# rballester/tntorch

Hardware: AMD Instinct MI355X
Metric: TT rounding 64^8 rank-64 -> rank-32 (round_tt rmax=32), cores/s, resident batch of 4096 trains per GPU (higher is better)
Workload: dtype f32

## Files before the change

include/ttround_hip.h:

```cpp
#ifndef TTROUND_HIP_H
#define TTROUND_HIP_H

#include <stdint.h>

#ifdef __cplusplus
extern "C" {
#endif

#define TTR_F32 0
#define TTR_F64 1

#define TTR_OK 0
#define TTR_E_INVALID (-1)
#define TTR_E_UNSUPPORTED (-2)
#define TTR_E_HIP (-3)
#define TTR_E_WORKSPACE (-4)

#define TTR_SCALE_NONE 0
#define TTR_SCALE_MUL 1
#define TTR_SCALE_DIV 2

#define TTR_EIG_RAW 0
#define TTR_EIG_REF 1
#define TTR_EIG_MATCH_DIAG 2
// ... 163 lines not shown
                   const void* sigma, int64_t stride_sigma, int left_ortho,
                   void* left, int64_t ldl, int64_t strideL,
                   void* right, int64_t ldr, int64_t strideR, void* stream);

int ttr_pow2_normalize(int dtype, int64_t count, int64_t batch, const void* x, int64_t stride_x,
                       void* out, int64_t stride_out, int32_t* e_out, int32_t* expo_acc, void* stream);

int ttr_scale_batch(int dtype, int64_t count, int64_t batch, const void* x, int64_t stride_x,
                    const void* scale, int64_t stride_scale, const int32_t* expo, int expo_sign,
                    void* out, int64_t stride_out, void* stream);

int64_t ttr_orth_fixup_workspace_bytes(int dtype, int64_t r, int64_t n, int64_t batch, int64_t elem_stride);
int ttr_orth_fixup(int dtype, int64_t r, int64_t n, int64_t batch, void* X, int64_t vec_stride, int64_t elem_stride,
                   int64_t strideX, const void* sigma, int64_t stride_sigma, double dead_rel, const int32_t* rank_dev,
                   void* workspace, int64_t workspace_bytes, void* stream);

#define TTR_ALG_SVD 0
#define TTR_ALG_EIG 1
int64_t ttr_round_tt_workspace_bytes(int dtype, int64_t N, const int64_t* shapes, const int64_t* rcap, int64_t batch,
                                     int eps_mode);
int ttr_round_tt(int dtype, int64_t N, const int64_t* shapes, int64_t batch, const void* const* cores_in, const int64_t* rcap,
                 int algorithm, int eps_mode, double eps, double flat_thr, int use_eigh_top, void* const* cores_out,
                 int32_t* ranks_dev, int32_t* zero_flag_dev, void* workspace, int64_t workspace_bytes, void* stream);

#define TTR_PROF_GEMM 0
#define TTR_PROF_QR_FACTOR 1
#define TTR_PROF_QR_APPLY 2
#define TTR_PROF_EIGH 3
#define TTR_PROF_MISC 4
#define TTR_PROF_ROTGRAM 5
#define TTR_PROF_PROJECT 6
#define TTR_PROF_ROWGRAM 7
#define TTR_PROF_NKINDS 8
int ttr_debug_set_qr_stamps(void* device_buffer);
#define TTR_KNOB_QR_PANEL 0
#define TTR_KNOB_BJ_INNER_SWEEPS 1
#define TTR_KNOB_GEMM_BIG 2
#define TTR_KNOB_QR_STAMP_BX 3
#define TTR_KNOB_QR_STAMP_BY 4
#define TTR_KNOB_QR_F64_NW4 5
#define TTR_KNOB_QR_RANK_SKIP 6
#define TTR_KNOB_QR_PACK 7
#define TTR_KNOB_RANK_NOISE_FLOOR 9
#define TTR_KNOB_ORTH_ROUNDS 10
#define TTR_KNOB_JACOBI_LIVE_WAVE 11
#define TTR_KNOB_ORTH_V2 12
#define TTR_KNOB_QR_INTERLEAVE 13
#define TTR_KNOB_SWEEP_STAGGER 14
#define TTR_KNOB_ORTH_SPLIT 15
#define TTR_KNOB_QR_STAGGER 16
#define TTR_KNOB_QR_PACK_PRE 17
#define TTR_KNOB_EIGH_BIG_OCC 18
#define TTR_KNOB_EIGH_SMALL 8
int ttr_debug_set_knob(int knob, int value);
int ttr_prof_enable(int on);
int ttr_prof_collect(double* ms, int64_t* launches);
int ttr_prof_collect_work(double* flops, double* bytes);


int64_t ttr_gather_chain_workspace_bytes(int dtype, int64_t nmodes, const int64_t* ranks, const int64_t* sizes, int64_t P,
                                         int64_t batch);
int ttr_gather_chain(int dtype, int64_t nmodes, int64_t batch, int64_t P, const int64_t* ranks, const int64_t* sizes,
                     const void* const* cores, const int64_t* core_strides, int idx_dtype, const void* const* idx,
                     const int64_t* idx_strides, void* out, int64_t stride_ob, int64_t stride_or, int64_t stride_op,
                     int64_t stride_oc, int64_t direct_max_points, void* oob_flag, void* workspace, int64_t workspace_bytes,
                     void* stream);

int ttr_gather_step(int dtype, int64_t P, int64_t rows_x, int64_t r, int64_t rn, int64_t I, const void* X, int64_t ldx,
                    const void* xrow, const void* G, int64_t gr, int64_t gi, int64_t gj, const void* idx, void* Y, int64_t ldy,
                    void* oob_flag, void* stream);

int64_t ttr_maxvol_workspace_bytes(int dtype, int64_t N, int64_t r, int64_t batch);
int ttr_maxvol(int dtype, int64_t batch, int64_t N, int64_t r, const void* A, int64_t stride_ab, double tol, int64_t max_iters,
               void* index, void* C, int64_t stride_cb, void* status, void* workspace, int64_t workspace_bytes, void* stream);

int64_t ttr_als_normal_groups(int64_t r0, int64_t r1);
int ttr_als_normal(int dtype, int64_t ntasks, int64_t r0, int64_t r1, const void* L, int64_t ldl, const void* R, int64_t ldr,
                   const void* w, const void* y, const void* perm, const void* task_begin, const void* task_end, void* Gp,
                   void* hp, void* stream);
int ttr_spd_solve(int dtype, int64_t n_items, int64_t K, const void* Gp, const void* hp, const void* part_off, int64_t part_base,
                  void* X, int64_t inner, int64_t s_item, int64_t s_a, int64_t s_b, void* Gsum, void* hsum, void* status,
                  const void* counts, void* stream);
int ttr_pinv_finish(int dtype, int64_t n_items, int64_t K, const void* V, const void* sigma, const void* t, const void* status,
                    void* X, int64_t inner, int64_t s_item, int64_t s_a, int64_t s_b, void* stream);

int64_t ttr_gather_grad_stage_rows(int dtype, int64_t r0, int64_t r1);
int64_t ttr_gather_grad_workspace_bytes(int dtype, int64_t ntasks, int64_t r0, int64_t r1);
int ttr_gather_grad(int dtype, int64_t I, int64_t ntasks, int64_t r0, int64_t r1, const void* L, int64_t ldl, const void* R,
                    int64_t ldr, const void* perm, const void* task_begin, const void* task_end, const void* task_off, void* dG,
                    void* workspace, int64_t workspace_bytes, void* stream);

int ttr_sparse_keys(int64_t P, int64_t N, const void* X, int64_t sx0, int64_t sx1, const void* shape, void* key, void* flag,
                    void* stream);
int ttr_sparse_levels(int64_t P, int64_t N, const void* X, int64_t sx0, int64_t sx1, const void* perm, void* lev, void* flag,
                      void* stream);
int64_t ttr_sparse_group_workspace_bytes(int64_t nb, int64_t I);
int ttr_sparse_group(int64_t nb, int64_t I, const void* blk_i, void* ilist, void* iptr, void* workspace, int64_t workspace_bytes,
                     void* stream);
int64_t ttr_sparse_gram_parts(int dtype, int64_t r, int64_t I, int64_t nb);
int64_t ttr_sparse_gram_workspace_bytes(int dtype, int64_t r, int64_t I, int64_t nb);
int ttr_sparse_gram(int dtype, int64_t r, int64_t I, int64_t nb, int64_t C, const void* colptr, const void* blk_i,
                    const void* blkcol, const void* ilist, const void* iptr, const void* V, int64_t ldv, void* G, int64_t ldg,
                    void* workspace, int64_t workspace_bytes, void* stream);
int ttr_sparse_project(int dtype, int64_t r, int64_t I, int64_t q, int64_t nb, int64_t C, const void* colptr, const void* blk_i,
                       const void* V, int64_t ldv, const void* U, int64_t su_row, int64_t su_col, void* W, int64_t ldw,
                       void* stream);
// ... 100 lines not shown
```

tntorch_amd/csrc/detail/ttr_internal.h:

```cpp
#pragma once
#include <type_traits>

#include "../ttr_common.h"

namespace ttr {

int gemm_dispatch(int dtype, int transA, int transB, int64_t M, int64_t N, int64_t K, const void* A, int64_t lda,
                  int64_t strideA, const void* B, int64_t ldb, int64_t strideB, void* C, int64_t ldc, int64_t strideC,
                  const void* rs, int64_t stride_rs, int rs_mode, const void* cs, int64_t stride_cs, int cs_mode,
                  int64_t batch, void* ws, int64_t ws_bytes, hipStream_t stream, int axpby = 0, double alpha = 1.0,
                  double beta = 0.0);
int64_t gemm_workspace_bytes(int dtype, int64_t M, int64_t N, int64_t K, int64_t batch);
int krp_contract_dispatch(int dtype, int64_t P, int64_t J, int64_t Q, int64_t R, const void* Tn, const void* B,
                          int64_t ldb, void* out, hipStream_t stream);
int hadamard_dispatch(int dtype, int64_t count, const void* a, const void* b, void* out, hipStream_t stream);
int core_kron_dispatch(int dtype, int64_t B, int64_t R1, int64_t S1, int64_t I, int64_t R2, int64_t S2, const void* a,
                       const void* c, void* out, hipStream_t stream);
int qr_factor_dispatch(int dtype, int64_t m, int64_t n, int64_t batch, const void* A, int64_t lda, int64_t strideA,
                       void* R, int64_t ldr, int64_t strideR, void* ws, int64_t ws_bytes, hipStream_t stream, int64_t a_cs = 1,
                       int32_t* expo_acc = nullptr);
int qr_apply_dispatch(int dtype, int64_t m, int64_t n, int64_t batch, void* ws, int64_t ws_bytes, const void* C,
                      int64_t ldc, int64_t strideC, int64_t kc, void* Out, int64_t ldo, int64_t strideO,
                      hipStream_t stream, int64_t o_cs = 1);
int64_t qr_workspace_bytes(int dtype, int64_t m, int64_t n, int64_t batch);
// ... 23 lines not shown
                        hipStream_t stream);
int bj_apply_dispatch(int dtype, int64_t b, int64_t npairs, int64_t items, void* G, int64_t ldg, int64_t strideG, void* V,
                      int64_t ldv, int64_t strideV, const int32_t* pair_tab, const void* W, const int32_t* ctrl, double* offsq,
                      hipStream_t stream);
int bj_control_dispatch(int dtype, int64_t items, int32_t* ctrl, double* state, const void* gnorm, int relative, double tol,
                        hipStream_t stream);
int64_t eigsel_scratch_bytes(int dtype, int64_t n, int64_t batch);
int eigsel_max_n();
int64_t tridiag_workspace_bytes(int dtype, int64_t n, int64_t batch);
int tridiag_dispatch(int dtype, int64_t n, int64_t batch, void* A, int64_t lda, int64_t strideA, void* d, void* e, void* tau,
                     void* ws, hipStream_t stream);
int eigsel_dispatch(int dtype, int64_t n, int64_t batch, int64_t k, const void* d, const void* e, void* lam, void* Z, void* scratch,
                    hipStream_t stream);
int tridiag_back_dispatch(int dtype, int64_t n, int64_t batch, int64_t k, const void* A, int64_t lda, int64_t strideA, const void* tau,
                          void* Z, hipStream_t stream);
int64_t eigh_workspace_bytes(int dtype, int64_t n, int64_t batch);
int eigh_max_n(int dtype);
int eigh_max_n_lds(int dtype);

int sweep_gram_parts(int64_t n, int64_t batch);
int sweep_gram_dispatch(int dtype, int64_t R, int64_t n, int64_t batch, const void* Mx, int64_t ldm, int64_t strideM,
                        const void* V1, int64_t ldv1, int64_t strideV1, void* G, int64_t nsplit, hipStream_t stream,
                        const int32_t* skip = nullptr, const int32_t* rows32 = nullptr);
int sweep_project_dispatch(int dtype, int64_t R, int64_t n, int64_t ro, int64_t batch, const void* Mx, int64_t ldm,
                           int64_t strideM, const void* V1, int64_t ldv1, int64_t strideV1, const void* V2, int64_t ldv2,
                           int64_t strideV2, const void* sigma, int64_t stride_sigma, int scale_right, void* right,
                           int64_t ldr, int64_t strideR, void* left, int64_t ldl, int64_t strideL, hipStream_t stream,
                           const int32_t* rows32 = nullptr);
int64_t qr_pushed_flag_offset(int dtype, int64_t I, int64_t n, int64_t batch);

int64_t colgram_workspace_bytes(int dtype, int64_t rows, int64_t n, int64_t batch);
int colgram_dispatch(int dtype, int64_t rows, int64_t n, int64_t batch, const void* Mx, int64_t ldm, int64_t strideM,
                     const void* V1, int64_t ldv1, int64_t strideV1, void* G, void* ws, int64_t ws_bytes, hipStream_t stream,
                     const int32_t* skip = nullptr);
int colproject_dispatch(int dtype, int64_t rows, int64_t n, int64_t ro, int64_t batch, const void* Mx, int64_t ldm,
                        int64_t strideM, const void* V1, int64_t ldv1, int64_t strideV1, const void* V2, int64_t ldv2,
                        int64_t strideV2, const void* sigma, int64_t stride_sigma, int left_ortho, void* left, int64_t ldl,
                        int64_t strideL, void* right, int64_t ldr, int64_t strideR, hipStream_t stream);

extern long long* g_qr_dbg;
extern int g_qr_variant;
extern int g_bj_inner_sweeps;
extern int g_gemm_big;
extern int g_qr_dbg_bx, g_qr_dbg_by;
extern int g_qr_f64_nw4;
extern int g_rank_skip_c;
extern int g_qr_pack;
extern int g_qr_interleave;
extern int g_qr_stagger;
extern int g_qr_pack_pre;
extern int g_qr_l1_idle;
extern int g_eigh_big_occ;
extern int g_sweep_stagger;
extern int g_rank_noise_c;
extern int g_jacobi_live_wave;
extern int g_eigh_small;
extern int g_orth_rounds, g_orth_v2, g_orth_split;

double* work_census_dev();

inline bool dtype_ok(int dtype) { return dtype == TTR_F32 || dtype == TTR_F64; }
inline int64_t elem_size(int dtype) { return dtype == TTR_F32 ? 4 : 8; }

template <typename F>
auto by_dtype(int dtype, F&& f) -> decltype(f(float{})) {
  if (dtype == TTR_F32) return f(float{});
  return f(double{});
}

inline bool contiguous(const int64_t* shape, const int64_t* strides, int nd) {
  int64_t want = 1;
  for (int d = nd - 1; d >= 0; --d) {
    if (shape[d] != 1 && strides[d] != want) return false;
    want *= shape[d];
  }
  return true;
}

inline bool aligned16(const void* p) { return ((uintptr_t)p & 15) == 0; }
inline int64_t align256(int64_t x) { return (x + 255) & ~int64_t(255); }

inline dim3 capped_grid(int64_t blocks) {
  const int64_t cap = 1 << 20;
  return dim3((unsigned)(blocks < cap ? blocks : cap));
}

template <typename T, typename F>
void by_pack_width(bool wide, F&& f) {
  if (wide) f(std::integral_constant<int, 16 / (int)sizeof(T)>{});
  else f(std::integral_constant<int, 1>{});
}

inline int core_check(const char* who, int dtype, int64_t R, int64_t I, int64_t C, const void* X, const int64_t* x_strides,
                      const void* out, const char* out_name, bool rest = true) {
  TTR_REQUIRE(dtype_ok(dtype), TTR_E_INVALID, "%s: bad dtype %d", who, dtype);
  TTR_REQUIRE(R >= 1 && I >= 1 && C >= 1, TTR_E_INVALID, "%s: bad sizes R = %lld, I = %lld, C = %lld", who, (long long)R, (long long)I,
              (long long)C);
  TTR_REQUIRE(X && x_strides && out && rest, TTR_E_INVALID, "%s: null pointer", who);
  TTR_REQUIRE(X != out, TTR_E_INVALID, "%s: X and %s must be different buffers", who, out_name);
  const int64_t xs[3] = {R, I, C};
  TTR_REQUIRE(contiguous(xs, x_strides, 3), TTR_E_UNSUPPORTED, "%s: X must be contiguous", who);
  TTR_REQUIRE((double)R * (double)I * (double)C < 9.0e18 / 64.0, TTR_E_UNSUPPORTED, "%s: core too large", who);
  return TTR_OK;
}

inline int strided_y_check(const char* who, int64_t R, int64_t I, int64_t C, const int64_t* y_strides, int64_t* sr, int64_t* si) {
// ... 10 lines not shown
```

tntorch_amd/csrc/ttr_api.hip:

```cpp
#include <stdarg.h>

#include <mutex>
#include <vector>

#include "detail/ttr_internal.h"

namespace ttr {

static thread_local std::string g_err;

void set_error(const char* fmt, ...) {
  char buf[512];
  va_list ap;
  va_start(ap, fmt);
  vsnprintf(buf, sizeof(buf), fmt, ap);
  va_end(ap);
  g_err = buf;
}

int hip_fail(hipError_t e, const char* what) {
  set_error("HIP error %d (%s) in %s", (int)e, hipGetErrorString(e), what);
  return TTR_E_HIP;
}

// ... 485 lines not shown
}

int ttr_krp_contract(int dtype, int64_t P, int64_t J, int64_t Q, int64_t R, const void* T, const void* B, int64_t ldb,
                     void* out, void* stream) {
  TTR_REQUIRE(dtype_ok(dtype), TTR_E_INVALID, "ttr_krp_contract: bad dtype %d", dtype);
  TTR_REQUIRE(P >= 0 && J >= 1 && Q >= 0 && R >= 1 && ldb >= R, TTR_E_INVALID, "ttr_krp_contract: bad sizes");
  if (P == 0 || Q == 0) return TTR_OK;
  TTR_REQUIRE(T && B && out, TTR_E_INVALID, "ttr_krp_contract: null pointer");
  return krp_contract_dispatch(dtype, P, J, Q, R, T, B, ldb, out, (hipStream_t)stream);
}

int ttr_hadamard(int dtype, int64_t count, const void* a, const void* b, void* out, void* stream) {
  TTR_REQUIRE(dtype_ok(dtype), TTR_E_INVALID, "ttr_hadamard: bad dtype %d", dtype);
  TTR_REQUIRE(count >= 0, TTR_E_INVALID, "ttr_hadamard: negative count");
  if (count == 0) return TTR_OK;
  TTR_REQUIRE(a && b && out, TTR_E_INVALID, "ttr_hadamard: null pointer");
  return hadamard_dispatch(dtype, count, a, b, out, (hipStream_t)stream);
}

int ttr_core_kron(int dtype, int64_t batch, int64_t R1, int64_t S1, int64_t I, int64_t R2, int64_t S2, const void* a,
                  const void* c, void* out, void* stream) {
  TTR_REQUIRE(dtype_ok(dtype), TTR_E_INVALID, "ttr_core_kron: bad dtype %d", dtype);
  TTR_REQUIRE(batch >= 0 && R1 >= 1 && S1 >= 1 && I >= 1 && R2 >= 1 && S2 >= 1, TTR_E_INVALID, "ttr_core_kron: bad sizes");
  if (batch == 0) return TTR_OK;
  TTR_REQUIRE(a && c && out, TTR_E_INVALID, "ttr_core_kron: null pointer");
  return core_kron_dispatch(dtype, batch, R1, S1, I, R2, S2, a, c, out, (hipStream_t)stream);
}

int ttr_debug_set_qr_stamps(void* device_buffer) {
  g_qr_dbg = (long long*)device_buffer;
  return TTR_OK;
}

int ttr_debug_set_knob(int knob, int value) {
  switch (knob) {
    case TTR_KNOB_QR_STAMP_BX:
      g_qr_dbg_bx = value;
      return TTR_OK;
    case TTR_KNOB_QR_STAMP_BY:
      g_qr_dbg_by = value;
      return TTR_OK;
    case TTR_KNOB_EIGH_SMALL:
      TTR_REQUIRE(value >= 0 && value <= 3, TTR_E_INVALID, "ttr_debug_set_knob: small-eigensolver switch %d outside [0, 3]", value);
      g_eigh_small = value;
      return TTR_OK;
    case TTR_KNOB_ORTH_SPLIT:
      TTR_REQUIRE(value >= 0 && value <= 65535, TTR_E_INVALID, "ttr_debug_set_knob: orth split threshold %d outside [0, 65535]", value);
      g_orth_split = value;
      return TTR_OK;
    case TTR_KNOB_SWEEP_STAGGER:
      TTR_REQUIRE(value >= 0 && value <= 2, TTR_E_INVALID, "ttr_debug_set_knob: stagger mode %d outside [0, 2]", value);
      g_sweep_stagger = value;
      return TTR_OK;
    case TTR_KNOB_EIGH_BIG_OCC:
      TTR_REQUIRE(value == 0 || value == 2 || value == 3, TTR_E_INVALID, "ttr_debug_set_knob: eigensolver occupancy %d not in {0, 2, 3}", value);
      g_eigh_big_occ = value;
      return TTR_OK;
    case TTR_KNOB_QR_PACK_PRE:
      TTR_REQUIRE(value >= 0 && value <= 3, TTR_E_INVALID, "ttr_debug_set_knob: pack-flag switch %d outside [0, 3]", value);
      g_qr_pack_pre = value & 1;
      g_qr_l1_idle = (value & 2) ? 0 : 1;
      return TTR_OK;
    case TTR_KNOB_QR_STAGGER:
      TTR_REQUIRE(value >= 0 && value <= 1024, TTR_E_INVALID, "ttr_debug_set_knob: stagger of %d kilo-cycles outside [0, 1024]", value);
      g_qr_stagger = value;
      return TTR_OK;
    case TTR_KNOB_QR_INTERLEAVE:
      TTR_REQUIRE(value >= 0 && value <= 1, TTR_E_INVALID, "ttr_debug_set_knob: interleave switch %d outside [0, 1]", value);
      g_qr_interleave = value;
      return TTR_OK;
    case TTR_KNOB_ORTH_V2:
      TTR_REQUIRE(value >= 0 && value <= 2, TTR_E_INVALID, "ttr_debug_set_knob: orth_fixup variant %d outside [0, 2]", value);
      g_orth_v2 = value;
      return TTR_OK;
    case TTR_KNOB_JACOBI_LIVE_WAVE:
      TTR_REQUIRE(value >= 0 && value <= 1, TTR_E_INVALID, "ttr_debug_set_knob: pass-2 Jacobi switch %d outside [0, 1]", value);
      g_jacobi_live_wave = value;
      return TTR_OK;
    case TTR_KNOB_ORTH_ROUNDS:
      TTR_REQUIRE(value >= 1 && value <= 4, TTR_E_INVALID, "ttr_debug_set_knob: %d rounds outside [1, 4]", value);
      g_orth_rounds = value;
      return TTR_OK;
    case TTR_KNOB_RANK_NOISE_FLOOR:
      TTR_REQUIRE(value >= 0 && value <= 1024, TTR_E_INVALID, "ttr_debug_set_knob: rank-rule noise floor %d outside [0, 1024]", value);
      g_rank_noise_c = value;
      return TTR_OK;
    case TTR_KNOB_QR_PACK:
      TTR_REQUIRE(value >= 0 && value <= 3, TTR_E_INVALID, "ttr_debug_set_knob: packing switch %d outside [0, 3]", value);
      g_qr_pack = value;
      return TTR_OK;
    case TTR_KNOB_QR_RANK_SKIP:
      TTR_REQUIRE(value >= 0 && value <= 4096, TTR_E_INVALID, "ttr_debug_set_knob: rank-skip factor %d outside [0, 4096]", value);
      g_rank_skip_c = value;
      return TTR_OK;
    case TTR_KNOB_QR_F64_NW4:
      TTR_REQUIRE(value >= 0 && value <= 7, TTR_E_INVALID, "ttr_debug_set_knob: 4-wave block switch %d outside [0, 7]", value);
      g_qr_f64_nw4 = value;
      return TTR_OK;
    case TTR_KNOB_GEMM_BIG:
      TTR_REQUIRE(value >= 0 && value <= 1, TTR_E_INVALID, "ttr_debug_set_knob: big-tile GEMM switch %d outside [0, 1]", value);
      g_gemm_big = value;
      return TTR_OK;
    case TTR_KNOB_BJ_INNER_SWEEPS:
      TTR_REQUIRE(value >= 0 && value <= 64, TTR_E_INVALID, "ttr_debug_set_knob: %d inner sweeps outside [0, 64]", value);
      g_bj_inner_sweeps = value;
      return TTR_OK;
// ... 57 lines not shown
```

tntorch_amd/csrc/ttr_sweep.hip:

```cpp
#include <type_traits>

#include "detail/ttr_internal.h"

namespace ttr {

constexpr int KLD = 80;

template <typename T>
struct SweepArgs {
  int R;
  int64_t n;
  const T* M;
  int64_t ldm, strideM;
  const T* V1;
  int64_t ldv1, strideV1;
  T* G;
  int nsplit;
  const int32_t* skip;
  const int32_t* rows32;
  const T* V2;
  int64_t ldv2, strideV2;
  const T* sigma;
  int64_t stride_sigma;
  int ro;
// ... 103 lines not shown
#pragma unroll
      for (int ks = 0; ks < 16; ++ks) {
        const int k = 4 * ks + g;
        a[ks] = (k < Rl && c0 + cl < p.n) ? Mp[(int64_t)k * p.ldm + c0 + cl] : T(0);
      }
    };
    const int64_t nsteps = ce > cb + wave ? (ce - cb - wave + 3) / 4 : 0;
    const int64_t rot = (p.stagger >= 2 && nsteps > 1) ? (int64_t)(b % nsteps) : 0;
    auto step_c = [&](int64_t sidx) { int64_t sq = sidx + rot; if (sq >= nsteps) sq -= nsteps; return cb + wave + 4 * sq; };
    T a[16], an[16];
    if (nsteps > 0) load_cols(step_c(0), a);
    for (int64_t sidx = 0; sidx < nsteps; ++sidx) {
      const bool more = sidx + 1 < nsteps;
      if (more) load_cols(step_c(sidx + 1), an);
      Acc mw[4];
#pragma unroll
      for (int t = 0; t < 4; ++t) {
        mw[t] = M::zero();
#pragma unroll
        for (int ks = 0; ks < 16; ++ks) mw[t] = M::mma(a[ks], Vl[(4 * ks + g) * KLD + 16 * t + cl], mw[t]);
      }
      gram_update(mw);
      if (more) {
#pragma unroll
        for (int ks = 0; ks < 16; ++ks) a[ks] = an[ks];
      }
    }
  }
  __syncthreads();
#pragma unroll
  for (int i = 0; i < 10; ++i)
#pragma unroll
    for (int r = 0; r < 4; ++r) smem[(wave * 10 + i) * 256 + lane * 4 + r] = G[i][r];
  __syncthreads();
  T* __restrict__ Gout = p.G + ((int64_t)b * p.nsplit + split) * R * R;
  for (int idx = tid; idx < 10 * 256; idx += kThreads) {
    const int tile = idx >> 8, e = idx & 255, ln = e >> 2, r = e & 3;
    const T v = (smem[idx] + smem[2560 + idx]) + (smem[5120 + idx] + smem[7680 + idx]);
    int ti = 0, rem = tile;
    while (rem >= 4 - ti) { rem -= 4 - ti; ++ti; }
    const int tj = ti + rem;
    const int row = 16 * ti + M::row(ln, r), col = 16 * tj + (ln & 15);
    if (row < R && col < R) {
      Gout[row * R + col] = v;
      if (ti != tj) Gout[col * R + row] = v;
    }
  }
}

constexpr int V1LD = 82;
constexpr int UBLK = 16 * V1LD;
__device__ __forceinline__ int urow(int k) { return (k >> 4) * UBLK + (k & 15) * KLD; }

template <typename T>
__global__ __launch_bounds__(kThreads, (sizeof(T) == 4 ? 4 : 1)) void project_kernel(SweepArgs<T> p) {
  using M = Mfma<T>;
  using Acc = typename M::Acc;
  constexpr int V2LD = 72;
  __shared__ __attribute__((aligned(16))) T V2l[64 * V2LD];
  __shared__ __attribute__((aligned(16))) T V1l[64 * V1LD];
  T* Ul = V1l;
  __shared__ T isg[64];
  const int tid = threadIdx.x, lane = tid & 63, wave = tid >> 6, cl = lane & 15, g = lane >> 4;
  const int64_t b = blockIdx.y;
  const int split = blockIdx.x;
  const T* __restrict__ Mp = p.M + b * p.strideM;
  const int R = p.R, ro = p.ro;
  const int nt = (ro + 15) / 16;
  const T* __restrict__ V2 = p.V2 + b * p.strideV2;
  const T* __restrict__ sg = p.sigma ? p.sigma + b * p.stride_sigma : nullptr;
  T* __restrict__ Lo = (p.left && split == 0) ? p.left + b * p.strideL : nullptr;
  for (int idx = tid; idx < 64 * 64; idx += kThreads) {
    const int m = idx >> 6, i = idx & 63;
    V2l[m * V2LD + i] = (m < R && i < ro) ? V2[(int64_t)m * p.ldv2 + i] : T(0);
  }
  if (tid < 64) {
    T sc = T(1);
    if (p.scale_right && sg && tid < ro) {
      const T x = sg[tid];
      sc = (fabs((double)x) < (double)Num<T>::tiny()) ? T(0) : T(1) / x;
    }
    isg[tid] = sc;
  }
  if (p.V1) {
    const T* __restrict__ V1 = p.V1 + b * p.strideV1;
    for (int idx = tid; idx < 64 * 64; idx += kThreads) {
      const int k = idx >> 6, m = idx & 63;
      V1l[k * V1LD + m] = (k < R && m < R) ? V1[(int64_t)k * p.ldv1 + m] : T(0);
    }
    __syncthreads();
    Acc u0 = M::zero(), u1 = M::zero(), u2 = M::zero(), u3 = M::zero();
#pragma unroll
    for (int ks = 0; ks < 16; ++ks) {
      const T a = V1l[(16 * wave + cl) * V1LD + 4 * ks + g];
      u0 = M::mma(a, V2l[(4 * ks + g) * V2LD + cl], u0);
      u1 = M::mma(a, V2l[(4 * ks + g) * V2LD + 16 + cl], u1);
      u2 = M::mma(a, V2l[(4 * ks + g) * V2LD + 32 + cl], u2);
      u3 = M::mma(a, V2l[(4 * ks + g) * V2LD + 48 + cl], u3);
    }
#pragma unroll
    for (int r = 0; r < 4; ++r) {
      T* dst = Ul + urow(16 * wave + M::row(lane, r)) + cl;
      dst[0] = u0[r];
      dst[16] = u1[r];
      dst[32] = u2[r];
      dst[48] = u3[r];
    }
  } else {
// ... 39 lines not shown
#pragma unroll
        for (int u = 0; u < SL; ++u) bm[u][ks] = x.v[u];
      }
#pragma unroll
      for (int t = 0; t < 4; ++t) {
        if (t < nt) {
          Acc acc[SL];
#pragma unroll
          for (int u = 0; u < SL; ++u) acc[u] = M::zero();
#pragma unroll
          for (int ks = 0; ks < NK; ++ks) {
            const T af = Ul[urow(4 * ks + g) + 16 * t + cl];
#pragma unroll
            for (int u = 0; u < SL; ++u) acc[u] = M::mma(af, bm[u][ks], acc[u]);
          }
#pragma unroll
          for (int r = 0; r < 4; ++r) {
            const int row = 16 * t + M::row(lane, r);
            if (row < ro && lim > 0) {
              const T sc = isg[row];
              T* dst = Ro + (int64_t)row * p.ldr + col;
              if (al && lim >= SL) {
                typedef T VT __attribute__((ext_vector_type(SL)));
                VT o;
#pragma unroll
                for (int u = 0; u < SL; ++u) o[u] = acc[u][r] * sc;
                *reinterpret_cast<VT*>(dst) = o;
              } else {
#pragma unroll
                for (int u = 0; u < SL; ++u)
                  if (u < lim) dst[u] = acc[u][r] * sc;
              }
            }
          }
        }
      }
    }
  };
  using I2 = std::integral_constant<int, 2>;
  using I4 = std::integral_constant<int, 4>;
  using I8 = std::integral_constant<int, 8>;
  using I16 = std::integral_constant<int, 16>;
  if (Rl <= 32) {
#ifdef TTR_PROJECT_WIDE
    if (al4) main_loop(I8{}, I4{});
    else
#endif
      main_loop(I8{}, I2{});
  } else {
    main_loop(I16{}, I2{});
  }
  (void)al4;
}

constexpr int CLD = 68;

template <typename T>
struct ColArgs {
  int64_t rows;
  int n;
  const T* M;
  int64_t ldm, strideM;
  const T* V1;
  int64_t ldv1, strideV1;
  T* G;
  int nsplit;
  const int32_t* skip;
  const T* V2;
  int64_t ldv2, strideV2;
  const T* sigma;
  int64_t stride_sigma;
  int ro;
  int left_ortho;
  T* left;
  int64_t ldl, strideL;
  T* right;
  int64_t ldr, strideR;
};

template <typename T, bool ROT>
__global__ __launch_bounds__(kThreads, (sizeof(T) == 4 ? (ROT ? 3 : 4) : 1)) void colgram_kernel(ColArgs<T> p) {
  using M = Mfma<T>;
  using Acc = typename M::Acc;
  constexpr int RED = 4 * 10 * 256;
  constexpr int VSZ = 64 * CLD;
  __shared__ __attribute__((aligned(16))) T smem[RED > VSZ ? RED : VSZ];
  T* Vl = smem;
  const int tid = threadIdx.x, lane = tid & 63, wave = tid >> 6, cl = lane & 15, g = lane >> 4;
  const int64_t b = blockIdx.y;
  if (p.skip && p.skip[b] != 0) return;
  const int split = blockIdx.x;
  const T* __restrict__ Mp = p.M + b * p.strideM;
  const int n = p.n;
  if constexpr (ROT) {
    const T* __restrict__ V1 = p.V1 + b * p.strideV1;
    for (int idx = tid; idx < 64 * 64; idx += kThreads) {
      const int k = idx >> 6, j = idx & 63;
      Vl[k * CLD + j] = (k < n && j < n) ? V1[(int64_t)k * p.ldv1 + j] : T(0);
    }
    __syncthreads();
  }
  Acc G[10];
#pragma unroll
  for (int i = 0; i < 10; ++i) G[i] = M::zero();
  int64_t cb, ce;
  split_range((p.rows + 15) / 16, p.nsplit, split, cb, ce);
// ... 253 lines not shown

int colgram_dispatch(int dtype, int64_t rows, int64_t n, int64_t batch, const void* Mx, int64_t ldm, int64_t strideM,
                     const void* V1, int64_t ldv1, int64_t strideV1, void* G, void* ws, int64_t ws_bytes, hipStream_t stream,
                     const int32_t* skip) {
  TTR_REQUIRE(n >= 1 && n <= 64, TTR_E_UNSUPPORTED, "ttr_colgram: %lld columns (the fused kernels hold <= 64)", (long long)n);
  if (dtype == TTR_F32) return colgram_typed<float>(rows, n, batch, Mx, ldm, strideM, V1, ldv1, strideV1, G, ws, ws_bytes, stream, skip);
  return colgram_typed<double>(rows, n, batch, Mx, ldm, strideM, V1, ldv1, strideV1, G, ws, ws_bytes, stream, skip);
}

template <typename T>
static int colproject_typed(int64_t rows, int64_t n, int64_t ro, int64_t batch, const void* Mx, int64_t ldm, int64_t strideM,
                            const void* V1, int64_t ldv1, int64_t strideV1, const void* V2, int64_t ldv2, int64_t strideV2,
                            const void* sigma, int64_t stride_sigma, int left_ortho, void* left, int64_t ldl,
                            int64_t strideL, void* right, int64_t ldr, int64_t strideR, hipStream_t stream) {
  ColArgs<T> p{};
  p.rows = rows; p.n = (int)n; p.M = (const T*)Mx; p.ldm = ldm; p.strideM = strideM;
  p.V1 = (const T*)V1; p.ldv1 = ldv1; p.strideV1 = strideV1;
  p.V2 = (const T*)V2; p.ldv2 = ldv2; p.strideV2 = strideV2;
  p.sigma = (const T*)sigma; p.stride_sigma = stride_sigma; p.ro = (int)ro; p.left_ortho = left_ortho;
  p.left = (T*)left; p.ldl = ldl; p.strideL = strideL;
  p.right = (T*)right; p.ldr = ldr; p.strideR = strideR;
  p.nsplit = col_split(rows, batch);
  ProfScope prof(TTR_PROF_PROJECT, stream);
  for (int64_t b0 = 0; b0 < batch; b0 += 65535) {
    const int64_t nb = batch - b0 < 65535 ? batch - b0 : 65535;
    ColArgs<T> q = p;
    q.M = p.M + b0 * strideM;
    if (V1) q.V1 = p.V1 + b0 * strideV1;
    q.V2 = p.V2 + b0 * strideV2;
    if (sigma) q.sigma = p.sigma + b0 * stride_sigma;
    q.left = p.left + b0 * strideL;
    if (right) q.right = p.right + b0 * strideR;
    if (q.V1) hipLaunchKernelGGL((colproject_kernel<T, true>), dim3((unsigned)p.nsplit, (unsigned)nb), dim3(kThreads), 0, stream, q);
    else hipLaunchKernelGGL((colproject_kernel<T, false>), dim3((unsigned)p.nsplit, (unsigned)nb), dim3(kThreads), 0, stream, q);
  }
  TTR_HIP_CHECK(hipGetLastError());
  return TTR_OK;
}

int colproject_dispatch(int dtype, int64_t rows, int64_t n, int64_t ro, int64_t batch, const void* Mx, int64_t ldm,
                        int64_t strideM, const void* V1, int64_t ldv1, int64_t strideV1, const void* V2, int64_t ldv2,
                        int64_t strideV2, const void* sigma, int64_t stride_sigma, int left_ortho, void* left, int64_t ldl,
                        int64_t strideL, void* right, int64_t ldr, int64_t strideR, hipStream_t stream) {
  TTR_REQUIRE(n >= 1 && n <= 64 && ro >= 1 && ro <= n, TTR_E_UNSUPPORTED,
              "ttr_colproject: %lld columns / %lld kept (the fused kernel holds <= 64 columns)", (long long)n, (long long)ro);
  if (dtype == TTR_F32)
    return colproject_typed<float>(rows, n, ro, batch, Mx, ldm, strideM, V1, ldv1, strideV1, V2, ldv2, strideV2, sigma,
                                   stride_sigma, left_ortho, left, ldl, strideL, right, ldr, strideR, stream);
  return colproject_typed<double>(rows, n, ro, batch, Mx, ldm, strideM, V1, ldv1, strideV1, V2, ldv2, strideV2, sigma,
                                  stride_sigma, left_ortho, left, ldl, strideL, right, ldr, strideR, stream);
}

int g_sweep_stagger = 1;

static int pick_split(int64_t n, int64_t batch) {
  const int64_t chunks = (n + 31) / 32;
  int64_t want = (2048 + batch - 1) / batch;
  int64_t maxs = chunks / 8;
  if (maxs < 1) maxs = 1;
  int64_t s = want < maxs ? want : maxs;
  if (s > 64) s = 64;
  return (int)(s < 1 ? 1 : s);
}

int sweep_gram_parts(int64_t n, int64_t batch) { return pick_split(n, batch); }

template <typename T>
static int gram_typed(int64_t R, int64_t n, int64_t batch, const void* Mx, int64_t ldm, int64_t strideM, const void* V1,
                      int64_t ldv1, int64_t strideV1, void* G, int64_t nsplit, hipStream_t stream, const int32_t* skip,
                      const int32_t* rows32) {
  SweepArgs<T> p{};
  p.skip = skip;
  p.rows32 = rows32;
  p.R = (int)R; p.n = n; p.M = (const T*)Mx; p.ldm = ldm; p.strideM = strideM;
  p.V1 = (const T*)V1; p.ldv1 = ldv1; p.strideV1 = strideV1;
  p.G = (T*)G; p.nsplit = (int)nsplit;
  p.stagger = g_sweep_stagger;
  if (work_census_on()) {
    const double s = (double)sizeof(T), sym = 10.0 / 16.0;
    auto gr = [&](double Re) { return 2.0 * Re * Re * (double)n * sym + (V1 ? 2.0 * (double)R * Re * (double)n : 0.0); };
    const double fl[4] = {gr((double)R), gr(R > 32 ? 32.0 : (double)R), 0.0, 0.0};
    const double by[4] = {s * R * (double)n, s * (R > 32 ? 32.0 : (double)R) * (double)n, 0.0, 0.0};
    work_items(V1 ? TTR_PROF_ROTGRAM : TTR_PROF_ROWGRAM, rows32, skip, batch, fl, by, stream);
  }
  ProfScope prof(V1 ? TTR_PROF_ROTGRAM : TTR_PROF_ROWGRAM, stream);
  for (int64_t b0 = 0; b0 < batch; b0 += 65535) {
    const int64_t nb = batch - b0 < 65535 ? batch - b0 : 65535;
    SweepArgs<T> q = p;
    q.M = p.M + b0 * strideM;
    if (V1) q.V1 = p.V1 + b0 * strideV1;
    q.G = p.G + b0 * nsplit * R * R;
    if (skip) q.skip = skip + b0;
    if (rows32) q.rows32 = rows32 + b0;
    const dim3 grid((unsigned)nsplit, (unsigned)nb);
    if (V1) hipLaunchKernelGGL((rotgram_kernel<T, false>), grid, dim3(kThreads), 0, stream, q);
    else hipLaunchKernelGGL((rotgram_kernel<T, true>), grid, dim3(kThreads), 0, stream, q);
  }
  TTR_HIP_CHECK(hipGetLastError());
  return TTR_OK;
}

int sweep_gram_dispatch(int dtype, int64_t R, int64_t n, int64_t batch, const void* Mx, int64_t ldm, int64_t strideM,
                        const void* V1, int64_t ldv1, int64_t strideV1, void* G, int64_t nsplit, hipStream_t stream,
                        const int32_t* skip, const int32_t* rows32) {
  TTR_REQUIRE(R >= 1 && R <= 64, TTR_E_UNSUPPORTED, "ttr_rowgram / ttr_rotgram: %lld rows (the fused kernels hold <= 64)",
              (long long)R);
  TTR_REQUIRE(nsplit >= 1 && nsplit <= 65535, TTR_E_INVALID, "ttr_rowgram / ttr_rotgram: bad split %lld", (long long)nsplit);
  if (dtype == TTR_F32) return gram_typed<float>(R, n, batch, Mx, ldm, strideM, V1, ldv1, strideV1, G, nsplit, stream, skip, rows32);
  return gram_typed<double>(R, n, batch, Mx, ldm, strideM, V1, ldv1, strideV1, G, nsplit, stream, skip, rows32);
}

template <typename T>
static int project_typed(int64_t R, int64_t n, int64_t ro, int64_t batch, const void* Mx, int64_t ldm, int64_t strideM,
                         const void* V1, int64_t ldv1, int64_t strideV1, const void* V2, int64_t ldv2, int64_t strideV2,
                         const void* sigma, int64_t stride_sigma, int scale_right, void* right, int64_t ldr,
                         int64_t strideR, void* left, int64_t ldl, int64_t strideL, hipStream_t stream, const int32_t* rows32) {
  SweepArgs<T> p{};
  p.rows32 = rows32;
  p.R = (int)R; p.n = n; p.M = (const T*)Mx; p.ldm = ldm; p.strideM = strideM;
  p.V1 = (const T*)V1; p.ldv1 = ldv1; p.strideV1 = strideV1;
  p.V2 = (const T*)V2; p.ldv2 = ldv2; p.strideV2 = strideV2;
  p.sigma = (const T*)sigma; p.stride_sigma = stride_sigma; p.ro = (int)ro; p.scale_right = scale_right;
  p.right = (T*)right; p.ldr = ldr; p.strideR = strideR;
  p.left = (T*)left; p.ldl = ldl; p.strideL = strideL;
  p.nsplit = pick_split(n, batch);
  p.stagger = g_sweep_stagger;
  if (work_census_on()) {
    const double s = (double)sizeof(T), Re = R > 32 ? 32.0 : (double)R;
    const double fl[4] = {2.0 * R * (double)ro * (double)n, 2.0 * Re * (double)ro * (double)n, 0.0, 0.0};
    const double by[4] = {s * (R + ro) * (double)n, s * (Re + ro) * (double)n, 0.0, 0.0};
    work_items(TTR_PROF_PROJECT, rows32, nullptr, batch, fl, by, stream);
  }
  ProfScope prof(TTR_PROF_PROJECT, stream);
  for (int64_t b0 = 0; b0 < batch; b0 += 65535) {
    const int64_t nb = batch - b0 < 65535 ? batch - b0 : 65535;
    SweepArgs<T> q = p;
    q.M = p.M + b0 * strideM;
    if (V1) q.V1 = p.V1 + b0 * strideV1;
    q.V2 = p.V2 + b0 * strideV2;
    if (sigma) q.sigma = p.sigma + b0 * stride_sigma;
    q.right = p.right + b0 * strideR;
    if (left) q.left = p.left + b0 * strideL;
    if (rows32) q.rows32 = rows32 + b0;
    hipLaunchKernelGGL(project_kernel<T>, dim3((unsigned)p.nsplit, (unsigned)nb), dim3(kThreads), 0, stream, q);
  }
  TTR_HIP_CHECK(hipGetLastError());
  return TTR_OK;
}

int sweep_project_dispatch(int dtype, int64_t R, int64_t n, int64_t ro, int64_t batch, const void* Mx, int64_t ldm,
                           int64_t strideM, const void* V1, int64_t ldv1, int64_t strideV1, const void* V2, int64_t ldv2,
                           int64_t strideV2, const void* sigma, int64_t stride_sigma, int scale_right, void* right,
                           int64_t ldr, int64_t strideR, void* left, int64_t ldl, int64_t strideL, hipStream_t stream,
                           const int32_t* rows32) {
  TTR_REQUIRE(R >= 1 && R <= 64 && ro >= 1 && ro <= R, TTR_E_UNSUPPORTED,
              "ttr_project: %lld rows / %lld kept (the fused kernel holds <= 64 rows)", (long long)R, (long long)ro);
  if (dtype == TTR_F32)
    return project_typed<float>(R, n, ro, batch, Mx, ldm, strideM, V1, ldv1, strideV1, V2, ldv2, strideV2, sigma,
                                stride_sigma, scale_right, right, ldr, strideR, left, ldl, strideL, stream, rows32);
  return project_typed<double>(R, n, ro, batch, Mx, ldm, strideM, V1, ldv1, strideV1, V2, ldv2, strideV2, sigma,
                               stride_sigma, scale_right, right, ldr, strideR, left, ldl, strideL, stream, rows32);
}

}
```

Before: 1.438 million.

## Add lean rows32-specialized gram and project kernels with higher occupancy

Adds specialized fp32 kernels for batch items flagged rows32 (effective rank at most 32): a gram kernel that accumulates only the 32x32 block with a register prefetch pipeline, and a projection kernel that keeps only 32 columns of the rotation. Both declare launch bounds of 8 blocks per unit. The existing general kernels are still launched afterwards but skip the items the lean kernels already handled. The aim is to cut wasted MFMA work and register pressure on reduced-rank items, at the cost of an extra launch per stage and more code paths.

```diff
diff --git a/include/ttround_hip.h b/include/ttround_hip.h
--- a/include/ttround_hip.h
+++ b/include/ttround_hip.h
@@ -239,6 +239,7 @@
 #define TTR_KNOB_QR_PACK_PRE 17
 #define TTR_KNOB_EIGH_BIG_OCC 18
 #define TTR_KNOB_EIGH_SMALL 8
+#define TTR_KNOB_SWEEP_LEAN 19
 int ttr_debug_set_knob(int knob, int value);
 int ttr_prof_enable(int on);
 int ttr_prof_collect(double* ms, int64_t* launches);
diff --git a/tntorch_amd/csrc/detail/ttr_internal.h b/tntorch_amd/csrc/detail/ttr_internal.h
--- a/tntorch_amd/csrc/detail/ttr_internal.h
+++ b/tntorch_amd/csrc/detail/ttr_internal.h
@@ -99,6 +99,7 @@
 extern int g_qr_l1_idle;
 extern int g_eigh_big_occ;
 extern int g_sweep_stagger;
+extern int g_sweep_lean;
 extern int g_rank_noise_c;
 extern int g_jacobi_live_wave;
 extern int g_eigh_small;
diff --git a/tntorch_amd/csrc/ttr_api.hip b/tntorch_amd/csrc/ttr_api.hip
--- a/tntorch_amd/csrc/ttr_api.hip
+++ b/tntorch_amd/csrc/ttr_api.hip
@@ -561,6 +561,10 @@
       TTR_REQUIRE(value >= 0 && value <= 2, TTR_E_INVALID, "ttr_debug_set_knob: stagger mode %d outside [0, 2]", value);
       g_sweep_stagger = value;
       return TTR_OK;
+    case TTR_KNOB_SWEEP_LEAN:
+      TTR_REQUIRE(value >= 0 && value <= 1, TTR_E_INVALID, "ttr_debug_set_knob: lean sweep switch %d outside [0, 1]", value);
+      g_sweep_lean = value;
+      return TTR_OK;
     case TTR_KNOB_EIGH_BIG_OCC:
       TTR_REQUIRE(value == 0 || value == 2 || value == 3, TTR_E_INVALID, "ttr_debug_set_knob: eigensolver occupancy %d not in {0, 2, 3}", value);
       g_eigh_big_occ = value;
diff --git a/tntorch_amd/csrc/ttr_sweep.hip b/tntorch_amd/csrc/ttr_sweep.hip
--- a/tntorch_amd/csrc/ttr_sweep.hip
+++ b/tntorch_amd/csrc/ttr_sweep.hip
@@ -179,8 +179,11 @@
 constexpr int UBLK = 16 * V1LD;
 __device__ __forceinline__ int urow(int k) { return (k >> 4) * UBLK + (k & 15) * KLD; }
 
-template <typename T>
+template <typename T, bool REST = false>
 __global__ __launch_bounds__(kThreads, (sizeof(T) == 4 ? 4 : 1)) void project_kernel(SweepArgs<T> p) {
+  if constexpr (REST) {
+    if (p.rows32[blockIdx.y] != 0) return;
+  }
   using M = Mfma<T>;
   using Acc = typename M::Acc;
   constexpr int V2LD = 72;
@@ -326,6 +329,243 @@
   }
   (void)al4;
 }
+
+constexpr int kLeanAhead = 3;
+
+template <typename T>
+__global__ __launch_bounds__(kThreads, 8) void rowgram_rows32_kernel(SweepArgs<T> p) {
+  using M = Mfma<T>;
+  using Acc = typename M::Acc;
+  __shared__ __attribute__((aligned(16))) T red[4 * 3 * 256];
+  static_assert(std::is_same<T, float>::value, "slab loads and the write-out below assume the fp32 accumulator layout");
+  const int tid = threadIdx.x, lane = tid & 63, cl = lane & 15, g = lane >> 4;
+  const int wave = __builtin_amdgcn_readfirstlane(tid >> 6);
+  const int64_t b = blockIdx.y;
+  if (p.rows32[b] == 0) return;
+  const int split = blockIdx.x;
+  const T* __restrict__ Mp = p.M + b * p.strideM;
+  Acc G[3];
+#pragma unroll
+  for (int i = 0; i < 3; ++i) G[i] = M::zero();
+  const bool al = ((p.ldm & 3) == 0) && ((reinterpret_cast<uintptr_t>(Mp) & (4 * sizeof(T) - 1)) == 0);
+  int64_t cb, ce;
+  split_range((p.n + 15) / 16, p.nsplit, split, cb, ce);
+  auto gram_update = [&](const Acc (&mw)[2]) {
+#pragma unroll
+    for (int r = 0; r < 4; ++r) G[0] = M::mma(mw[0][r], mw[0][r], G[0]);
+#pragma unroll
+    for (int r = 0; r < 4; ++r) G[1] = M::mma(mw[0][r], mw[1][r], G[1]);
+#pragma unroll
+    for (int r = 0; r < 4; ++r) G[2] = M::mma(mw[1][r], mw[1][r], G[2]);
+  };
+  const int64_t nsteps = ce > cb + wave ? (ce - cb - wave + 3) / 4 : 0;
+  const int64_t rot = (p.stagger >= 2 && nsteps > 1) ? (int64_t)(b % nsteps) : 0;
+  auto step_c = [&](int64_t sidx) { int64_t sq = sidx + rot; if (sq >= nsteps) sq -= nsteps; return cb + wave + 4 * sq; };
+  constexpr int NS = kLeanAhead + 1;
+  auto run = [&](auto WIDEC) {
+    constexpr bool WIDE = decltype(WIDEC)::value;
+    auto load_slab = [&](int64_t c, Acc (&mw)[2]) {
+      const int64_t col = c * 16 + 4 * g;
+#pragma unroll
+      for (int t = 0; t < 2; ++t) {
+        const T* src = Mp + (int64_t)(16 * t + cl) * p.ldm + col;
+        if constexpr (WIDE) {
+          mw[t] = *reinterpret_cast<const Acc*>(src);
+        } else {
+          const Pack<T, 4> x = load_pack<T, 4>(src, al, p.n - col);
+#pragma unroll
+          for (int r = 0; r < 4; ++r) mw[t][r] = x.v[r];
+        }
+      }
+    };
+    Acc slab[NS][2];
+    int64_t s0 = 0;
+    if (nsteps >= NS + kLeanAhead) {
+#pragma unroll
+      for (int d = 0; d < kLeanAhead; ++d) load_slab(step_c(d), slab[d]);
+      do {
+#pragma unroll
+        for (int u = 0; u < NS; ++u) {
+          load_slab(step_c(s0 + u + kLeanAhead), slab[(u + kLeanAhead) % NS]);
+          __builtin_amdgcn_sched_barrier(0);
+          gram_update(slab[u]);
+          __builtin_amdgcn_sched_barrier(0);
+        }
+        s0 += NS;
+      } while (s0 + NS + kLeanAhead <= nsteps);
+    } else {
+#pragma unroll
+      for (int d = 0; d < kLeanAhead; ++d)
+        if (d < nsteps) load_slab(step_c(d), slab[d]);
+    }
+    for (; s0 < nsteps; s0 += NS) {
+#pragma unroll
+      for (int u = 0; u < NS; ++u) {
+        const int64_t sidx = s0 + u;
+        if (sidx < nsteps) {
+          if (sidx + kLeanAhead < nsteps) load_slab(step_c(sidx + kLeanAhead), slab[(u + kLeanAhead) % NS]);
+          gram_update(slab[u]);
+        }
+      }
+    }
+  };
+  if (al && ce * 16 <= p.n) run(std::true_type{});
+  else run(std::false_type{});
+#pragma unroll
+  for (int i = 0; i < 3; ++i)
+#pragma unroll
+    for (int r = 0; r < 4; ++r) red[(wave * 3 + i) * 256 + lane * 4 + r] = G[i][r];
+  __syncthreads();
+  T* __restrict__ Gout = p.G + ((int64_t)b * p.nsplit + split) * 64 * 64;
+  for (int idx = tid; idx < 64 * 64; idx += kThreads) {
+    const int row = idx >> 6, col = idx & 63;
+    T v = T(0);
+    if (row < 32 && col < 32) {
+      const bool low = row >= 16 && col < 16;
+      const int i = (low ? col : row) & 15, j = (low ? row : col) & 15;
+      const int tile = (row >> 4) + (col >> 4);
+      const int e = tile * 256 + ((i >> 2) * 16 + j) * 4 + (i & 3);
+      v = (red[e] + red[768 + e]) + (red[1536 + e] + red[2304 + e]);
+    }
+    Gout[idx] = v;
+  }
+}
+
+constexpr int ULD = 48;
+
+template <typename T>
+__global__ __launch_bounds__(kThreads, 8) void project_rows32_kernel(SweepArgs<T> p) {
+  using M = Mfma<T>;
+  using Acc = typename M::Acc;
+  __shared__ __attribute__((aligned(16))) T Wl[64 * ULD];
+  __shared__ T isg[32];
+  static_assert(std::is_same<T, float>::value, "the store addresses below assume the fp32 accumulator layout");
+  const int tid = threadIdx.x, lane = tid & 63, cl = lane & 15, g = lane >> 4;
+  const int wave = __builtin_amdgcn_readfirstlane(tid >> 6);
+  const int64_t b = blockIdx.y;
+  if (p.rows32[b] == 0) return;
+  const int split = blockIdx.x;
+  const T* __restrict__ Mp = p.M + b * p.strideM;
+  const int ro = p.ro;
+  const int nt = (ro + 15) / 16;
+  const T* __restrict__ V2 = p.V2 + b * p.strideV2;
+  const T* __restrict__ sg = p.sigma ? p.sigma + b * p.stride_sigma : nullptr;
+  T* __restrict__ Lo = (p.left && split == 0) ? p.left + b * p.strideL : nullptr;
+  for (int idx = tid; idx < 64 * 32; idx += kThreads) {
+    const int m = idx >> 5, i = idx & 31;
+    Wl[m * ULD + i] = (i < ro) ? V2[(int64_t)m * p.ldv2 + i] : T(0);
+  }
+  if (tid < 32) {
+    T sc = T(1);
+    if (p.scale_right && sg && tid < ro) {
+      const T x = sg[tid];
+      sc = (fabs((double)x) < (double)Num<T>::tiny()) ? T(0) : T(1) / x;
+    }
+    isg[tid] = sc;
+  }
+  if (p.V1) {
+    const T* __restrict__ V1 = p.V1 + b * p.strideV1 + (int64_t)(16 * wave + cl) * p.ldv1 + g;
+    T a[16];
+#pragma unroll
+    for (int ks = 0; ks < 16; ++ks) a[ks] = V1[4 * ks];
+    __syncthreads();
+    Acc u0 = M::zero(), u1 = M::zero();
+#pragma unroll
+    for (int ks = 0; ks < 16; ++ks) {
+      u0 = M::mma(a[ks], Wl[(4 * ks + g) * ULD + cl], u0);
+      u1 = M::mma(a[ks], Wl[(4 * ks + g) * ULD + 16 + cl], u1);
+    }
+    __syncthreads();
+#pragma unroll
+    for (int r = 0; r < 4; ++r) {
+      T* dst = Wl + (16 * wave + M::row(lane, r)) * ULD + cl;
+      dst[0] = u0[r];
+      dst[16] = u1[r];
+    }
+  }
+  __syncthreads();
+  if (Lo) {
+    for (int idx = tid; idx < 64 * ro; idx += kThreads) {
+      const int k = idx / ro, i = idx - k * ro;
+      const T u = Wl[k * ULD + i];
+      Lo[(int64_t)k * p.ldl + i] = (p.scale_right && sg) ? u * sg[i] : u;
+    }
+  }
+  T af[2][8];
+#pragma unroll
+  for (int t = 0; t < 2; ++t)
+#pragma unroll
+    for (int ks = 0; ks < 8; ++ks) af[t][ks] = Wl[(4 * ks + g) * ULD + 16 * t + cl];
+  T* __restrict__ Ro = p.right + b * p.strideR;
+  const bool al = ((p.ldm & 1) == 0) && ((p.ldr & 1) == 0) && ((reinterpret_cast<uintptr_t>(Mp) & (2 * sizeof(T) - 1)) == 0) &&
+                  ((reinterpret_cast<uintptr_t>(Ro) & (2 * sizeof(T) - 1)) == 0);
+  int64_t cb, ce;
+  split_range((p.n + 31) / 32, p.nsplit, split, cb, ce);
+  const int64_t col_b = cb * 32, col_e = ce * 32 < p.n ? ce * 32 : p.n;
+  const int64_t nch = (col_e - col_b + 31) / 32;
+  const int64_t nsteps = nch > wave ? (nch - wave + 3) / 4 : 0;
+  const int64_t rot = (p.stagger && nsteps > 1) ? (int64_t)(b % nsteps) : 0;
+  const T* __restrict__ Mg = Mp + (int64_t)g * p.ldm;
+  T* __restrict__ Rg = Ro + (int64_t)M::row(lane, 0) * p.ldr;
+  typedef T VT __attribute__((ext_vector_type(2)));
+  auto step = [&](auto WHOLEC, const T* mk, T* rk, int64_t lim) {
+    constexpr bool WHOLE = decltype(WHOLEC)::value;
+    T bm[2][8];
+#pragma unroll
+    for (int ks = 0; ks < 8; ++ks) {
+      const T* src = mk + (int64_t)(4 * ks) * p.ldm;
+      if constexpr (WHOLE) {
+        const VT x = *reinterpret_cast<const VT*>(src);
+        bm[0][ks] = x[0];
+        bm[1][ks] = x[1];
+      } else {
+        const Pack<T, 2> x = load_pack<T, 2>(src, al, lim > 0 ? lim : 0);
+        bm[0][ks] = x.v[0];
+        bm[1][ks] = x.v[1];
+      }
+    }
+#pragma unroll
+    for (int t = 0; t < 2; ++t) {
+      if (t < nt) {
+        Acc acc[2] = {M::zero(), M::zero()};
+#pragma unroll
+        for (int ks = 0; ks < 8; ++ks) {
+#pragma unroll
+          for (int u = 0; u < 2; ++u) acc[u] = M::mma(af[t][ks], bm[u][ks], acc[u]);
+        }
+#pragma unroll
+        for (int r = 0; r < 4; ++r) {
+          const int row = 16 * t + M::row(lane, r);
+          if (row < ro && (WHOLE || lim > 0)) {
+            const T sc = isg[row];
+            T* dst = rk + (int64_t)(16 * t + r) * p.ldr;
+            if (WHOLE || (al && lim >= 2)) {
+              VT o;
+              o[0] = acc[0][r] * sc;
+              o[1] = acc[1][r] * sc;
+              *reinterpret_cast<VT*>(dst) = o;
+            } else {
+              dst[0] = acc[0][r] * sc;
+              if (lim > 1) dst[1] = acc[1][r] * sc;
+            }
+          }
+        }
+      }
+    }
+  };
+  for (int64_t sidx = 0; sidx < nsteps; ++sidx) {
+    int64_t sq = sidx + rot;
+    if (sq >= nsteps) sq -= nsteps;
+    const int64_t cw = col_b + (wave + 4 * sq) * 32;
+    int64_t col = cw + 2 * cl;
+    asm volatile("" : "+v"(col));
+    const T* mk = Mg + col;
+    T* rk = Rg + col;
+    if (al && cw + 32 <= col_e) step(std::true_type{}, mk, rk, 2);
+    else step(std::false_type{}, mk, rk, col_e - col);
+  }
+}
+
 
 constexpr int CLD = 68;
 
@@ -685,6 +925,8 @@
 }
 
 int g_sweep_stagger = 1;
+int g_sweep_lean = 1;
+constexpr int64_t kLeanMinItems = 256;
 
 static int pick_split(int64_t n, int64_t batch) {
   const int64_t chunks = (n + 31) / 32;
@@ -726,6 +968,12 @@
     if (skip) q.skip = skip + b0;
     if (rows32) q.rows32 = rows32 + b0;
     const dim3 grid((unsigned)nsplit, (unsigned)nb);
+    if constexpr (std::is_same<T, float>::value) {
+      if (g_sweep_lean && !V1 && !skip && rows32 && R == 64 && nb >= kLeanMinItems) {
+        hipLaunchKernelGGL(rowgram_rows32_kernel<T>, grid, dim3(kThreads), 0, stream, q);
+        q.skip = q.rows32;
+      }
+    }
     if (V1) hipLaunchKernelGGL((rotgram_kernel<T, false>), grid, dim3(kThreads), 0, stream, q);
     else hipLaunchKernelGGL((rotgram_kernel<T, true>), grid, dim3(kThreads), 0, stream, q);
   }
@@ -775,7 +1023,16 @@
     q.right = p.right + b0 * strideR;
     if (left) q.left = p.left + b0 * strideL;
     if (rows32) q.rows32 = rows32 + b0;
-    hipLaunchKernelGGL(project_kernel<T>, dim3((unsigned)p.nsplit, (unsigned)nb), dim3(kThreads), 0, stream, q);
+    const dim3 grid((unsigned)p.nsplit, (unsigned)nb);
+    bool two = false;
+    if constexpr (std::is_same<T, float>::value) {
+      two = g_sweep_lean && rows32 && R == 64 && ro <= 32 && nb >= kLeanMinItems;
+      if (two) {
+        hipLaunchKernelGGL(project_rows32_kernel<T>, grid, dim3(kThreads), 0, stream, q);
+        hipLaunchKernelGGL((project_kernel<T, true>), grid, dim3(kThreads), 0, stream, q);
+      }
+    }
+    if (!two) hipLaunchKernelGGL((project_kernel<T, false>), grid, dim3(kThreads), 0, stream, q);
   }
   TTR_HIP_CHECK(hipGetLastError());
   return TTR_OK;
```

Result: faster. 1.459 million (median of 6 runs) (+1.5%).
